# earth-insights/ZoomEarth

Hardware: AMD Instinct MI355X
Metric: questions/sec end-to-end, ZoomEarth-3B on 5000px tiles (higher is better)
Workload: dtype bf16

## Files before the change

### include/zoomearth.h

```cpp
#ifndef ZOOMEARTH_H
#define ZOOMEARTH_H

#include <stddef.h>
#include <stdint.h>

#ifdef __cplusplus
extern "C" {
#endif

typedef struct ze_engine ze_engine;

typedef enum {
    ZE_OK = 0,
    ZE_ERR_INVALID = -1,
    ZE_ERR_HIP = -2,
    ZE_ERR_NOMEM = -3,
    ZE_ERR_NOTFOUND = -4,
    ZE_ERR_MISMATCH = -5
} ze_status;

typedef enum { ZE_F32 = 0, ZE_F16 = 1, ZE_BF16 = 2 } ze_dtype;

#define ZE_MAX_FULLATT 16
#define ZE_MAX_EOS 4
// ... 199 lines not shown
int ze_weight_format(ze_engine* e);

int ze_op_linear(ze_engine* e, const void* a_bf16, const void* w_bf16, const void* bias_bf16, void* c_bf16, int M,
                 int N, int K, int act, void* stream);
int ze_op_gemm(ze_engine* e, int launcher, int epi, const void* a_bf16, int lda, const void* w_bf16, int ldw, const void* bias_bf16,
               const void* r_bf16, int ldr, void* c, int ldc, const int32_t* c_rows, int M, int N, int K, void* stream);
int ze_op_rmsnorm(ze_engine* e, const void* x_bf16, const void* weight_bf16, void* y_bf16, int rows, int cols,
                  float eps, void* stream);
int ze_op_token_logprob(ze_engine* e, const void* logits_bf16, int rows, int vocab, int ld, const int32_t* targets,
                        float* out, void* stream);
int ze_op_score_detail(ze_engine* e, const void* logits_bf16, int rows, int vocab, int ld, const int32_t* targets, int top_n,
                       float* out_logprob, float* out_entropy, int32_t* out_rank, int32_t* out_top_ids, float* out_top_logprobs,
                       void* stream);
int ze_op_attention(ze_engine* e, const void* q, const void* k, const void* v, void* o, int T, int heads,
                    int kv_heads, int D, const int32_t* cu_seqlens, int n_seg, int causal, void* stream);

int ze_op_window_gather(ze_engine* e, const float* pixel_values, const int32_t* grid_thw, int n_images, void* out_bf16, void* stream);
int ze_op_window_scatter(ze_engine* e, const void* x_bf16, int cols, const int32_t* grid_thw, int n_images, void* out_bf16,
                         void* stream);
int ze_op_vision_rope(ze_engine* e, void* qkv_bf16, const int32_t* grid_thw, int n_images, int window_order, void* stream);
int ze_op_embed_scatter(ze_engine* e, const int32_t* input_ids, int len, const void* image_embeds, int n_image_rows, void* out_bf16,
                        void* stream);
int ze_op_mrope_kv(ze_engine* e, int seq, int layer, void* qkv_bf16, int T, const int32_t* position_ids, int past, void* stream);
int ze_op_rope_kv_decode(ze_engine* e, const int32_t* seqs, int n, int layer, void* qkv_bf16, void* stream);
int ze_op_kv_read(ze_engine* e, int seq, int layer, int start, int n, void* out_k, void* out_v, void* stream);

int ze_seq_set_speculation(ze_engine* e, int seq, int k, int min_ngram, int max_ngram, const int32_t* prompt_ids, int n_prompt, void* stream);
int ze_chain_spec_stats(ze_engine* e, int seq, int* steps, int* drafted, int* accepted, void* stream);
int ze_op_spec_draft(ze_engine* e, const int32_t* hist_ids, const int32_t* hist_lens, int rows, int ld, int k, int min_ngram,
                     int max_ngram, int32_t* out_draft, int32_t* out_len, void* stream);
int ze_op_spec_accept(ze_engine* e, const float* logits, int n_chains, int vocab, int ld, int k, const int32_t* draft,
                      const int32_t* draft_len, uint8_t* seen, const float* repetition_penalty, const int32_t* room, int ignore_eos,
                      int32_t* out_tokens, int32_t* out_count, int32_t* out_finished, void* stream);
int ze_op_decode_rows(ze_engine* e, int seq, const int32_t* tokens, int r, float* out_logits, void* stream);
int ze_op_attn_decode(ze_engine* e, const int32_t* seqs, int n, int layer, const void* qkv_bf16, void* out_bf16, void* stream);
int ze_op_attn_decode_single(ze_engine* e, int seq, int layer, const void* qkv_bf16, void* out_bf16, void* stream);
int ze_op_gemv(ze_engine* e, int epi, const void* w_bf16, const void* w8, const void* scale8, const void* x_bf16, const void* norm_w,
               float eps, const void* bias_bf16, int act8, int N, int K, void* out_bf16, float* out_f32, const uint8_t* seen,
               float penalty, int32_t* out_token, int seq, int layer, const void* embed, int token, void* embed_out, void* stream);
int ze_op_logits_rows(ze_engine* e, const void* w_bf16, const void* norm_w, float eps, const void* x_bf16, float* out_f32, int n, int N,
                      int K, void* stream);

int ze_op_numeric_helpers(ze_engine* e, const float* x, const float* y, uint32_t* out, uint32_t* out2, int n, void* stream);

int ze_profile_decode_kernel(ze_engine* e, int which, int iters, float* avg_us, double* bytes_per_launch,
                             void* stream);
int ze_profile_batch_kernel(ze_engine* e, int which, int n, int iters, float* avg_us, double* bytes_per_launch,
                            void* stream);
int ze_profile_prefill_kernel(ze_engine* e, int which, int rows, int iters, float* avg_us, double* flops_per_launch,
                              void* stream);
int ze_profile_prefill_layer(ze_engine* e, int rows, int layers_run, float avg_us[4], double flops[4], void* stream);
int ze_tune(int knob, int value);
int ze_phase_timers(ze_engine* e, int enable, int reset, float out_ms[5]);

#ifdef __cplusplus
}
#endif
#endif
```

### zoomearth_amd/_lib.py

```python
from __future__ import annotations

import ctypes as C
import os
import subprocess

_HERE = os.path.dirname(os.path.abspath(__file__))
LIB_PATH = os.environ.get("ZE_LIB_PATH") or os.path.join(_HERE, "libzoomearth_hip.so")
CSRC = os.path.join(_HERE, "csrc")

ZE_F32, ZE_F16, ZE_BF16 = 0, 1, 2
ZE_MAX_FULLATT, ZE_MAX_EOS = 16, 4


class ZeConfig(C.Structure):
    _fields_ = [
        ("vit_depth", C.c_int32), ("vit_hidden", C.c_int32), ("vit_heads", C.c_int32),
        ("vit_intermediate", C.c_int32), ("vit_out_hidden", C.c_int32),
        ("patch_size", C.c_int32), ("temporal_patch_size", C.c_int32), ("spatial_merge_size", C.c_int32),
        ("window_size", C.c_int32), ("in_channels", C.c_int32),
        ("n_fullatt", C.c_int32), ("fullatt_block_indexes", C.c_int32 * ZE_MAX_FULLATT),
        ("hidden", C.c_int32), ("layers", C.c_int32), ("heads", C.c_int32), ("kv_heads", C.c_int32),
        ("intermediate", C.c_int32), ("vocab", C.c_int32),
        ("rms_eps", C.c_float), ("rope_theta", C.c_float), ("mrope_section", C.c_int32 * 3),
        ("tie_word_embeddings", C.c_int32),
# ... 138 lines not shown
                                          C.POINTER(C.c_float), C.c_int, C.c_int, C.POINTER(C.c_int32), _P]),
    "ze_op_token_logprobs": (C.c_int, [_P, _P, C.c_int, C.c_int, C.c_int, _P, C.c_int, _P, _P, _P, _P]),
    "ze_seq_set_logit_adjust": (C.c_int, [_P, C.c_int, C.c_float, C.c_float, C.c_int, C.POINTER(C.c_int32), C.POINTER(C.c_float),
                                          C.c_int, _P]),
    "ze_op_logit_adjust": (C.c_int, [_P, _P, C.c_int, C.c_int, C.c_int, _P, _P, _P, _P, _P, _P, _P, _P, _P]),
    "ze_seq_set_token_rules": (C.c_int, [_P, C.c_int, C.c_int, C.POINTER(C.c_int32), C.c_int, C.POINTER(C.c_int32), C.c_int,
                                         C.POINTER(C.c_int32), C.c_int, _P]),
    "ze_op_token_rules": (C.c_int, [_P, _P, C.c_int, C.c_int, C.c_int, _P, _P, _P, _P, _P, _P, _P, _P, _P, _P, _P, _P]),
    "ze_grammar_create": (C.c_int, [_P, C.POINTER(C.c_uint16), C.c_int, C.POINTER(C.c_int16), C.c_int, C.POINTER(C.c_uint8),
                                    C.POINTER(C.c_int), _P]),
    "ze_grammar_destroy": (C.c_int, [_P, C.c_int]),
    "ze_seq_set_grammar": (C.c_int, [_P, C.c_int, C.c_int, C.c_int, _P]),
    "ze_chain_grammar_state": (C.c_int, [_P, C.c_int, C.POINTER(C.c_int), C.POINTER(C.c_int), _P]),
    "ze_op_grammar_mask": (C.c_int, [_P, C.c_int, _P, C.c_int, C.c_int, C.c_int, _P, _P, _P]),
    "ze_op_grammar_advance": (C.c_int, [_P, C.c_int, _P, _P, C.c_int, _P, _P]),
    "ze_weights_quantize_fp8": (C.c_int, [_P, _P]),
    "ze_set_fp8_activations": (C.c_int, [_P, C.c_int]),
    "ze_op_quantize_fp8": (C.c_int, [_P, _P, C.c_int, C.c_int, _P, _P, _P]),
    "ze_weights_quantize_mxfp4": (C.c_int, [_P, _P]),
    "ze_op_quantize_mxfp4": (C.c_int, [_P, _P, C.c_int, C.c_int, _P, _P, _P]),
    "ze_op_gemv4": (C.c_int, [_P, C.c_int, _P, _P, _P, _P, C.c_float, _P, C.c_int, C.c_int, _P, _P, _P, C.c_float,
                              C.POINTER(C.c_int32), C.c_int, C.c_int, _P, C.c_int, _P, _P]),
    "ze_weight_format": (C.c_int, [_P]),
    "ze_op_linear_mx": (C.c_int, [_P, _P, _P, _P, _P, _P, _P, C.c_int, C.c_int, C.c_int, C.c_int, _P]),
    "ze_op_linear": (C.c_int, [_P, _P, _P, _P, _P, C.c_int, C.c_int, C.c_int, C.c_int, _P]),
    "ze_op_gemm": (C.c_int, [_P, C.c_int, C.c_int, _P, C.c_int, _P, C.c_int, _P, _P, C.c_int, _P, C.c_int, _P, C.c_int, C.c_int,
                             C.c_int, _P]),
    "ze_op_rmsnorm": (C.c_int, [_P, _P, _P, _P, C.c_int, C.c_int, C.c_float, _P]),
    "ze_op_attention": (C.c_int, [_P, _P, _P, _P, _P, C.c_int, C.c_int, C.c_int, C.c_int, C.POINTER(C.c_int32),
                                  C.c_int, C.c_int, _P]),
    "ze_op_window_gather": (C.c_int, [_P, _P, C.POINTER(C.c_int32), C.c_int, _P, _P]),
    "ze_op_window_scatter": (C.c_int, [_P, _P, C.c_int, C.POINTER(C.c_int32), C.c_int, _P, _P]),
    "ze_op_vision_rope": (C.c_int, [_P, _P, C.POINTER(C.c_int32), C.c_int, C.c_int, _P]),
    "ze_op_embed_scatter": (C.c_int, [_P, C.POINTER(C.c_int32), C.c_int, _P, C.c_int, _P, _P]),
    "ze_op_mrope_kv": (C.c_int, [_P, C.c_int, C.c_int, _P, C.c_int, C.POINTER(C.c_int32), C.c_int, _P]),
    "ze_op_rope_kv_decode": (C.c_int, [_P, C.POINTER(C.c_int32), C.c_int, C.c_int, _P, _P]),
    "ze_op_attn_decode": (C.c_int, [_P, C.POINTER(C.c_int32), C.c_int, C.c_int, _P, _P, _P]),
    "ze_op_attn_decode_single": (C.c_int, [_P, C.c_int, C.c_int, _P, _P, _P]),
    "ze_op_kv_read": (C.c_int, [_P, C.c_int, C.c_int, C.c_int, C.c_int, _P, _P, _P]),
    "ze_seq_set_speculation": (C.c_int, [_P, C.c_int, C.c_int, C.c_int, C.c_int, C.POINTER(C.c_int32), C.c_int, _P]),
    "ze_chain_spec_stats": (C.c_int, [_P, C.c_int, C.POINTER(C.c_int), C.POINTER(C.c_int), C.POINTER(C.c_int), _P]),
    "ze_op_spec_draft": (C.c_int, [_P, _P, _P, C.c_int, C.c_int, C.c_int, C.c_int, C.c_int, _P, _P, _P]),
    "ze_op_spec_accept": (C.c_int, [_P, _P, C.c_int, C.c_int, C.c_int, C.c_int, _P, _P, _P, _P, _P, C.c_int, _P, _P, _P, _P]),
    "ze_op_decode_rows": (C.c_int, [_P, C.c_int, C.POINTER(C.c_int32), C.c_int, _P, _P]),
    "ze_op_gemv": (C.c_int, [_P, C.c_int, _P, _P, _P, _P, _P, C.c_float, _P, C.c_int, C.c_int, C.c_int, _P, _P, _P, C.c_float,
                             C.POINTER(C.c_int32), C.c_int, C.c_int, _P, C.c_int, _P, _P]),
    "ze_op_logits_rows": (C.c_int, [_P, _P, _P, C.c_float, _P, _P, C.c_int, C.c_int, C.c_int, _P]),
    "ze_op_numeric_helpers": (C.c_int, [_P, _P, _P, _P, _P, C.c_int, _P]),
    "ze_profile_decode_kernel": (C.c_int, [_P, C.c_int, C.c_int, C.POINTER(C.c_float), C.POINTER(C.c_double), _P]),
    "ze_profile_batch_kernel": (C.c_int, [_P, C.c_int, C.c_int, C.c_int, C.POINTER(C.c_float), C.POINTER(C.c_double), _P]),
    "ze_profile_prefill_kernel": (C.c_int, [_P, C.c_int, C.c_int, C.c_int, C.POINTER(C.c_float), C.POINTER(C.c_double), _P]),
    "ze_profile_prefill_layer": (C.c_int, [_P, C.c_int, C.c_int, C.POINTER(C.c_float), C.POINTER(C.c_double), _P]),
    "ze_phase_timers": (C.c_int, [_P, C.c_int, C.c_int, C.POINTER(C.c_float)]),
    "ze_tune": (C.c_int, [C.c_int, C.c_int]),
}
EXPORTS = tuple(_SIGS)


def lib():
    global _lib
    if _lib is not None:
        return _lib
    if not os.path.exists(LIB_PATH):
        raise ImportError(
            f"{LIB_PATH} is missing: build it with `python -c 'import __graft_entry__ as g; g.build()'` "
            "(or `make -C zoomearth_amd/csrc`). zoomearth_amd has no CPU fallback.")
    try:
        import torch
    except Exception:
        pass
    handle = C.CDLL(LIB_PATH, mode=C.RTLD_GLOBAL)
    for name, (res, args) in _SIGS.items():
        fn = getattr(handle, name)
        fn.restype = res
        fn.argtypes = args
    _lib = handle
    return _lib


def check(code: int, engine=None):
    if code < 0:
        msg = lib().ze_last_error(engine)
        raise ZoomEarthError(code, msg.decode("utf-8", "replace") if msg else "")
    return code
```

### zoomearth_amd/csrc/ze_engine.h

```cpp
#pragma once
#include <algorithm>
#include <map>
#include <tuple>
#include <set>
#include <string>
#include <vector>

#include "ze_host.h"
#include "ze_kernels.h"

struct ze_linear {
    bf16_t* w = nullptr;
    bf16_t* bias = nullptr;
    int n = 0, k = 0, ld = 0;
    uint8_t* w8 = nullptr;
    float* scale8 = nullptr;
    int ld8 = 0;
    uint8_t* w4 = nullptr;
    uint8_t* scale4 = nullptr;
    bf16_t* wf = nullptr;
    bf16_t* wp = nullptr;
    bf16_t* bias_p = nullptr;
    uint8_t* wf8 = nullptr;
};
// ... 203 lines not shown
    size_t fe_tmp_bytes = 0, fe_img_bytes = 0, fe_coef_ints = 0;
    int* fe_coef_host = nullptr;
    hipEvent_t v_staged = nullptr, t_staged = nullptr;
    hipEvent_t fe_done = nullptr;
    bool fe_in_flight = false;

    bf16_t *vx = nullptr, *vh = nullptr, *vy = nullptr, *vqkv = nullptr, *vo = nullptr, *va = nullptr, *vz = nullptr,
           *vz2 = nullptr;
    float *vcos = nullptr, *vsin = nullptr;
    int *vperm = nullptr, *vinv = nullptr;
    int4* vtiles_win = nullptr;
    int4* vtiles_full = nullptr;
    int* v_host_ints = nullptr;
    float* v_host_f32 = nullptr;
    size_t v_host_ints_cap = 0, v_host_f32_cap = 0;

    bf16_t *th = nullptr, *ty = nullptr, *tqkv = nullptr, *to = nullptr, *ta = nullptr;
    int *tsrc = nullptr, *tpos = nullptr;
    int4* ttiles = nullptr;
    int* ttile_aux = nullptr;
    int* trow_aux = nullptr;
    int* tscore = nullptr;
    int prefill_rows = 0;
    int* t_host_ints = nullptr;
    size_t t_host_ints_cap = 0;
    int *xs_host = nullptr, *xs_dev = nullptr, *xt_host = nullptr, *xt_dev = nullptr;
    size_t xs_cap = 0, xt_cap = 0;
    int *xl_host = nullptr, *xl_dev = nullptr;
    size_t xl_cap = 0;
    hipEvent_t xs_staged = nullptr;

    bf16_t *dh = nullptr, *dq = nullptr, *dattn = nullptr, *dact = nullptr;
    float *dlogits = nullptr, *dpartial = nullptr, *dsample = nullptr;
    int max_splits = 64;
    int* d_host_ints = nullptr;
    unsigned* atickets = nullptr;
    unsigned bgraph_epoch = 0;
    float* gslab = nullptr;
    size_t gslab_floats = 0;
    int gticket_cap = 0;
    ze_gemm_ws gemm_ws() const { return ze_gemm_ws{gslab, gslab_floats, gtickets, gticket_cap}; }
    unsigned* gtickets = nullptr;
    float* pslab = nullptr;
    size_t pslab_floats = 0;
    unsigned* ptickets = nullptr;
    int pticket_cap = 0;
    ze_gemm_ws prefill_ws();
    bf16_t *bh = nullptr, *by = nullptr, *bqkv = nullptr, *bo = nullptr, *ba = nullptr;
    int* bseq = nullptr;
    float *blogits = nullptr, *bpartial = nullptr, *bsample = nullptr;
    ze_seq_dev* bstate_host = nullptr;
    std::map<ze_step_key, hipGraphExec_t> bgraphs;
    int live_parts = 0;

    bool timers_on = false;
    bool counted = false;
    struct ev_pair { int phase; hipEvent_t a, b; };
    std::vector<ev_pair> ev_used;
    std::vector<ev_pair> ev_free;
    float phase_ms[5] = {0, 0, 0, 0, 0};

    bf16_t* kc(int layer, int seq) const {
        return kcache + (((size_t)layer * cfg.max_seqs + seq) * cfg.kv_heads) * (size_t)cfg.max_ctx * head_dim;
    }
    bf16_t* vc(int layer, int seq) const {
        return vcache + (((size_t)layer * cfg.max_seqs + seq) * cfg.kv_heads) * (size_t)cfg.max_ctx * head_dim;
    }
};

#define ZE_TRY(x)               \
    do {                        \
        int _r = (x);           \
        if (_r != 0) return _r; \
    } while (0)
#define ZE_KCHECK() ZE_HIP(hipGetLastError())

extern unsigned ze_tune_epoch;
void ze_weights_changed(ze_engine* e);
int ze_engine_build_layout(ze_engine* e);
int ze_timer_begin(ze_engine* e, int phase, hipStream_t s);
void ze_timer_end(ze_engine* e, int handle, hipStream_t s);

template <typename T>
static int dev_alloc(ze_engine* e, T** p, size_t count, bool zero = true) {
    ZE_HIP(hipMalloc((void**)p, std::max<size_t>(count, 1) * sizeof(T)));
    if (zero) ZE_HIP(hipMemset(*p, 0, std::max<size_t>(count, 1) * sizeof(T)));
    return 0;
}
static inline int check_seq(ze_engine* e, int seq) {
    if (!e) return ze_fail(e, ZE_ERR_INVALID, "null engine");
    if (seq < 0 || seq >= e->cfg.max_seqs) return ze_fail(e, ZE_ERR_NOTFOUND, "sequence id out of range");
    return ZE_OK;
}

#pragma GCC visibility push(hidden)
int ze_requests_create(ze_engine* e);
void ze_requests_free(ze_engine* e);
void ze_requests_clear(ze_engine* e, int seq, hipStream_t s);
const float* ze_requests_rows(ze_engine* e, const float* logits, const int* seq_ids, int slot0, int n, hipStream_t s);
void ze_requests_logprobs(ze_engine* e, const float* logits, const int* seq_ids, int slot0, int n, hipStream_t s);
void ze_requests_after_token(ze_engine* e, const float* logits, const int* seq_ids, int slot0, int n, hipStream_t s);
int ze_check_filter(ze_engine* e, int top_k, float top_p, float min_p);
int ze_check_entropy_filter(ze_engine* e, float typical_p, float epsilon_cutoff, float eta_cutoff);
void ze_attach_filters(ze_engine* e, ze_sample_opts& so, bool batch);
float ze_penalty_of(const ze_engine* e, const ze_gen_params* p, int seq);
ze_sample_opts ze_sample_opts_of(ze_engine* e, const ze_gen_params* p, int slot, bool batch = false);
// ... 55 lines not shown
```

### zoomearth_amd/csrc/ze_forward.hip

```cpp
#include <math.h>
#include <cmath>
#include <string.h>

#include <algorithm>

#include "ze_engine.h"

extern int ze_gemv_knobs[24];

static int frontend_acquire(ze_engine* e) {
    if (e->fe_in_flight) {
        ZE_HIP(hipEventSynchronize(e->fe_done));
        e->fe_in_flight = false;
    }
    return ZE_OK;
}
static int frontend_release(ze_engine* e, hipStream_t s) {
    if (!e->fe_done) ZE_HIP(hipEventCreateWithFlags(&e->fe_done, hipEventDisableTiming));
    ZE_HIP(hipEventRecord(e->fe_done, s));
    e->fe_in_flight = true;
    return ZE_OK;
}
static int stage_acquire(ze_engine* e, hipEvent_t& ev) {
    if (ev) ZE_HIP(hipEventSynchronize(ev));
    return ZE_OK;
}
static int stage_release(ze_engine* e, hipEvent_t& ev, hipStream_t s) {
    if (!ev) ZE_HIP(hipEventCreateWithFlags(&ev, hipEventDisableTiming));
    ZE_HIP(hipEventRecord(ev, s));
    return ZE_OK;
}
static int crop_resize(ze_engine* e, const uint8_t* src, int src_h, int src_w, const int32_t box[4], uint8_t* dst,
                       int dst_h, int dst_w, hipStream_t s) {
    const int bx0 = box[0], by0 = box[1];
    const int bw = box[2] - box[0], bh = box[3] - box[1];
    if (bw <= 0 || bh <= 0 || dst_w <= 0 || dst_h <= 0) return ze_fail(e, ZE_ERR_INVALID, "empty crop box or output");
    const bool need_h = bw != dst_w, need_v = bh != dst_h;
    if (!need_h && !need_v) {
        ze_launch_crop(src, src_h, src_w, bx0, by0, dst, dst_h, dst_w, s);
        ZE_KCHECK();
        return ZE_OK;
    }
    ze_coeffs ch, cv;
    size_t ints = 0;
    if (need_h) {
        ze_bicubic_coeffs(bw, dst_w, &ch);
        ints += 2 * (size_t)dst_w + ch.kk.size();
    }
    if (need_v) {
        ze_bicubic_coeffs(bh, dst_h, &cv);
        ints += 2 * (size_t)dst_h + cv.kk.size();
    }
    if (ints > e->fe_coef_ints) return ze_fail(e, ZE_ERR_NOMEM, "bicubic coefficient table exceeds workspace");
    if (need_h && need_v && (size_t)bh * dst_w * 3 > e->fe_tmp_bytes)
        return ze_fail(e, ZE_ERR_NOMEM, "resize intermediate exceeds workspace (max_tile_side)");
    ZE_TRY(frontend_acquire(e));
    int* hp = e->fe_coef_host;
// ... 1100 lines not shown
static int op_sample(ze_engine* e, int seq, const float* logits, float repetition_penalty, const ze_sample_opts& so,
                     int index, int32_t* out_token, hipStream_t s) {
    ZE_TRY(check_seq(e, seq));
    if (!logits || !out_token) return ze_fail(e, ZE_ERR_INVALID, "null argument");
    if (index < 0 || index >= e->cfg.max_ctx) return ze_fail(e, ZE_ERR_INVALID, "index out of range");
    const ze_config& c = e->cfg;
    hipSetDevice(e->device);
    e->logits_fresh[seq] = 0;
    ZE_TRY(push_state(e, seq, s, 0, 0, 0));
    if (index) ze_launch_set_ints(&(e->st_dev + seq)->n_gen, &index, 1, s);
    ze_launch_sample(logits, c.vocab, e->seen + (size_t)seq * c.vocab, repetition_penalty, e->st_dev + seq, e->eos_dev,
                     c.n_eos, c.pad_token_id, 1, 0, e->out_tokens + (size_t)seq * c.max_ctx, e->dsample, so, s);
    ze_requests_logprobs(e, logits, nullptr, seq, 1, s);
    ZE_KCHECK();
    ZE_HIP(hipMemcpyAsync(out_token, e->out_tokens + (size_t)seq * c.max_ctx + index, sizeof(int), hipMemcpyDeviceToHost, s));
    ZE_HIP(hipStreamSynchronize(s));
    return ZE_OK;
}

extern "C" int ze_op_sample_greedy(ze_engine* e, int seq, const float* logits, float repetition_penalty,
                                   int32_t* out_token, void* stream) {
    return op_sample(e, seq, logits, repetition_penalty, ze_sample_opts{}, 0, out_token, (hipStream_t)stream);
}

extern "C" int ze_op_sample_temperature(ze_engine* e, int seq, const float* logits, float repetition_penalty,
                                        float temperature, uint64_t seed, int index, int32_t* out_token, void* stream) {
    if (!(temperature > 0.f)) return ze_fail(e, ZE_ERR_INVALID, "temperature must be positive");
    ze_sample_opts so;
    so.temperature = temperature;
    so.seed = seed;
    so.slot = seq;
    if (check_seq(e, seq) == 0) ze_attach_filters(e, so, false);
    return op_sample(e, seq, logits, repetition_penalty, so, index, out_token, (hipStream_t)stream);
}

template <typename F>
static int capture_step(ze_engine* e, F enqueue, hipGraphExec_t* exec) {
    hipStream_t cs;
    ZE_HIP(hipStreamCreateWithFlags(&cs, hipStreamNonBlocking));
    hipGraph_t graph = nullptr;
    int r = ZE_OK;
    if (hipStreamBeginCapture(cs, hipStreamCaptureModeThreadLocal) != hipSuccess)
        r = ze_fail(e, ZE_ERR_HIP, "hipStreamBeginCapture failed");
    if (r == ZE_OK) r = enqueue(cs);
    if (hipStreamEndCapture(cs, &graph) != hipSuccess && r == ZE_OK)
        r = ze_fail(e, ZE_ERR_HIP, "hipStreamEndCapture failed");
    if (r == ZE_OK && hipGraphInstantiate(exec, graph, nullptr, nullptr, 0) != hipSuccess)
        r = ze_fail(e, ZE_ERR_HIP, "hipGraphInstantiate failed");
    if (graph) hipGraphDestroy(graph);
    hipStreamDestroy(cs);
    return r;
}

static int first_token(ze_engine* e, int q, float pen, int ign, const ze_sample_opts& so, hipStream_t s) {
    const ze_config& c = e->cfg;
    const float* row = e->dlogits + (size_t)q * c.vocab;
    e->logits_fresh[q] = 0;
    ze_launch_sample(ze_requests_rows(e, row, nullptr, q, 1, s), c.vocab, e->seen + (size_t)q * c.vocab, pen, e->st_dev + q, e->eos_dev,
                     c.n_eos, c.pad_token_id, ign, 0, e->out_tokens + (size_t)q * c.max_ctx, e->dsample, so, s);
    ze_requests_after_token(e, row, nullptr, q, 1, s);
    ZE_KCHECK();
    return ZE_OK;
}

static int trim_at_eos(const ze_config& c, const int32_t* tokens, int n) {
    for (int i = 0; i < n; ++i)
        for (int k = 0; k < c.n_eos; ++k)
            if (tokens[i] == c.eos_token_ids[k]) return i + 1;
    return n;
}

extern "C" int ze_generate(ze_engine* e, int seq, const ze_gen_params* p, int32_t* out_tokens, int* n_out,
                           void* stream) {
    ZE_TRY(check_seq(e, seq));
    if (!p || !out_tokens || !n_out) return ze_fail(e, ZE_ERR_INVALID, "null argument");
    const ze_config& c = e->cfg;
    hipStream_t s = (hipStream_t)stream;
    hipSetDevice(e->device);
    int max_new = p->max_new_tokens;
    if (max_new <= 0) {
        *n_out = 0;
        return ZE_OK;
    }
    if (e->ctx_host[seq] + max_new - 1 > c.max_ctx) max_new = c.max_ctx - e->ctx_host[seq] + 1;
    if (max_new <= 0) return ze_fail(e, ZE_ERR_NOMEM, "sequence exceeds max_ctx");
    const float pen = ze_penalty_of(e, p, seq);
    const int ign = p->ignore_eos ? 1 : 0;
    const ze_sample_opts so = ze_sample_opts_of(e, p, seq);
    int32_t* dev_out = e->out_tokens + (size_t)seq * c.max_ctx;
    ze_seq_dev* st = e->st_dev + seq;

    const int t_s = ze_timer_begin(e, 4, s);
    const int r0 = first_token(e, seq, pen, ign, so, s);
    ze_timer_end(e, t_s, s);
    ZE_TRY(r0);

    hipGraphExec_t gexec = nullptr;
    if (p->use_graph && max_new > 1) {
        const ze_step_key key = ze_step_key_of(e, 0, seq, pen, ign, so);
        if (!e->graphs[seq] || !(e->graph_key[seq] == key)) {
            if (e->graphs[seq]) {
                hipGraphExecDestroy(e->graphs[seq]);
                e->graphs[seq] = nullptr;
            }
            ZE_TRY(capture_step(e, [&](hipStream_t cs) { return ze_enqueue_decode_step(e, seq, pen, ign, true, so, cs); }, &e->graphs[seq]));
            e->graph_key[seq] = key;
// ... 80 lines not shown
            q.kv_heads = c.kv_heads;
        }
        ZE_HIP(hipMemcpyAsync(e->qkv_epi_dev, host.data(), sizeof(ze_qkv_epi) * c.layers, hipMemcpyHostToDevice, s));
        ZE_HIP(hipStreamSynchronize(s));
        ZE_KCHECK();
    }
    if (ok && !wide) {
        const size_t per_layer = (size_t)(nqkv + 2 * ip) * H + (size_t)H * nq;
        const size_t total = per_layer * c.layers + (size_t)c.vocab * H;
        if (!e->arena_f) ZE_HIP(hipMalloc((void**)&e->arena_f, total * sizeof(bf16_t)));
        bf16_t* cur = e->arena_f;
        auto pack = [&](ze_linear& l, int rows, int cols, int rope_dim) {
            ze_launch_pack_fragments(l.w, l.ld, rows, cols, cur, s, rope_dim);
            l.wf = cur;
            cur += (size_t)rows * cols;
        };
        for (int li = 0; li < c.layers; ++li) {
            ze_text_layer& L = e->tl[li];
            pack(L.qkv, nqkv, H, hd);
            pack(L.o, H, nq, 0);
            pack(L.gate_up, 2 * ip, H, 0);
        }
        ze_launch_pack_fragments(e->lm_head, H, c.vocab, H, cur, s);
        e->lm_head_f = cur;
        for (int li = 0; li < c.layers; ++li) {
            ze_text_layer& L = e->tl[li];
            L.qkv.wf8 = L.o.wf8 = L.gate_up.wf8 = nullptr;
        }
        e->lm_head8.wf8 = nullptr;
        if (e->fp8_ready) {
            const bool head8 = e->lm_head8.w8 != nullptr;
            const size_t bytes = ((size_t)(nqkv + 2 * ip) * H + (size_t)H * nq) * c.layers + (head8 ? (size_t)c.vocab * H : 0);
            if (!e->arena_f8) ZE_HIP(hipMalloc((void**)&e->arena_f8, bytes));
            uint8_t* c8 = e->arena_f8;
            auto pack8 = [&](ze_linear& l, int rows, int cols, int rope_dim) {
                ze_launch_pack_fragments8(l.w8, l.ld8, rows, cols, c8, s, rope_dim);
                l.wf8 = c8;
                c8 += (size_t)rows * cols;
            };
            for (int li = 0; li < c.layers; ++li) {
                ze_text_layer& L = e->tl[li];
                pack8(L.qkv, nqkv, H, hd);
                pack8(L.o, H, nq, 0);
                pack8(L.gate_up, 2 * ip, H, 0);
            }
            if (head8) pack8(e->lm_head8, c.vocab, H, 0);
        }
        ZE_KCHECK();
    }
    e->frag_ready = true;
    return ZE_OK;
}

void set_live_parts(ze_engine* e, const int32_t* seqs, int n, int steps) {
    int mx = 0, ml = 0;
    for (int i = 0; i < n; ++i) {
        const int c = e->ctx_host[seqs[i]] + std::max(1, steps) + 1, sp = e->split_host[seqs[i]];
        mx = std::max(mx, e->ctx_host[seqs[i]]);
        ml = std::max(ml, (sp + 383) / 384 + (c - sp + 383) / 384);
    }
    e->live_parts = (mx + std::max(1, steps) + 1 + 191) / 192;
    e->live_parts_long = ml;
}

void upload_mates(ze_engine* e, const int32_t* seqs, int n, hipStream_t s) {
    std::vector<int> mate(n, -1);
    if (e->prefix_hints && ze_gemv_knobs[17] != 1) {
        std::map<long long, int> open;
        for (int i = 0; i < n; ++i) {
            const int q = seqs[i], sp = e->split_host[q];
            if (sp <= 0) continue;
            const int h = e->pfx_pushed[q];
            const int holder = (h != 0 && (h & 0xffff) >= sp) ? (h >> 16) : q;
            const long long key = ((long long)holder << 20) | (long long)sp;
            auto it = open.find(key);
            if (it == open.end()) open[key] = i;
            else {
                mate[i] = it->second;
                mate[it->second] = i;
                open.erase(it);
            }
        }
    }
    ze_launch_set_ints(e->bmate, mate.data(), n, s);
}

static int upload_batch(ze_engine* e, const int32_t* seqs, int n, hipStream_t s) {
    if (n <= 0 || n > e->cfg.max_seqs) return ze_fail(e, ZE_ERR_INVALID, "batch size out of range");
    if (n > 64 && !e->wide_regime())
        return ze_fail(e, ZE_ERR_INVALID, "more than 64 chains in a step of an engine pinned to the fragment kernels (ze_set_decode_regime)");
    for (int i = 0; i < n; ++i) {
        if (seqs[i] < 0 || seqs[i] >= e->cfg.max_seqs) return ze_fail(e, ZE_ERR_NOTFOUND, "sequence id out of range");
        for (int j = 0; j < i; ++j)
            if (seqs[j] == seqs[i]) return ze_fail(e, ZE_ERR_INVALID, "duplicate sequence id in a batch");
        if (e->ctx_host[seqs[i]] + 1 > e->cfg.max_ctx) return ze_fail(e, ZE_ERR_NOMEM, "sequence exceeds max_ctx");
    }
    ze_launch_set_ints(e->bseq, seqs, n, s);
    sync_prefix(e, seqs, n, s);
    upload_mates(e, seqs, n, s);
    return ZE_OK;
}

static bool attn_per_wave(const ze_engine* e) {
    const ze_config& c = e->cfg;
    const int wparts = (c.max_ctx + 191) / 192;
    return ze_gemv_knobs[8] != 2 && ze_gemv_knobs[11] == 0 && wparts <= std::max(e->max_splits, 8) && wparts <= 64 && e->head_dim == 128 &&
           c.heads / c.kv_heads <= 16;
}

static void launch_batch_attention(ze_engine* e, int li, int n, bool frag_out, hipStream_t s, const bf16_t* q_rows = nullptr,
                                   bf16_t* out_rows = nullptr) {
    const ze_config& c = e->cfg;
    const int hd = e->head_dim, nq = c.heads * hd, nqkv = nq + 2 * c.kv_heads * hd;
    const size_t seq_stride = (size_t)c.kv_heads * c.max_ctx * hd;
    const float scale = 1.0f / sqrtf((float)hd);
    const bf16_t* qb = q_rows ? q_rows : e->bqkv;
    bf16_t* ob = out_rows ? out_rows : e->bo;
    if (e->brow_off && !q_rows) {
// ... 128 lines not shown
    return false;
}

static int enqueue_decode_batch(ze_engine* e, int n, float penalty, int ignore_eos, int sample, const ze_sample_opts& so,
                                hipStream_t s) {
    const ze_config& c = e->cfg;
    ze_launch_embed_tokens_batch(e->st_dev, e->bseq, n, e->embed, e->bh, c.hidden, s);
    for (int li = 0; li < c.layers; ++li) {
        batch_norm(e, li, n, ZE_NORM_IN, s);
        batch_qkv(e, li, n, s);
        batch_attention(e, li, n, s);
        batch_o(e, li, n, s);
        batch_norm(e, li, n, ZE_NORM_POST, s);
        batch_gate_up(e, li, n, s);
        batch_down(e, li, n, s);
    }
    batch_norm(e, 0, n, ZE_NORM_FINAL, s);
    batch_lm_head(e, 0, n, s);
    ze_launch_sample_batch(sample ? ze_requests_rows(e, e->blogits, e->bseq, 0, n, s) : e->blogits, c.vocab, e->seen, penalty, e->st_dev,
                           e->bseq, n, e->eos_dev, c.n_eos, c.pad_token_id, ignore_eos, 1, sample, e->out_tokens, c.max_ctx, e->bsample,
                           e->bsample + (size_t)c.max_seqs * 2 * 128, so, s);
    if (sample) ze_requests_after_token(e, e->blogits, e->bseq, 0, n, s);
    ZE_KCHECK();
    return ZE_OK;
}

extern "C" int ze_decode_batch(ze_engine* e, const int32_t* seqs, int n, const int32_t* tokens, float* out_logits,
                               void* stream) {
    if (!e || !seqs) return ze_fail(e, ZE_ERR_INVALID, "null argument");
    const ze_config& c = e->cfg;
    hipStream_t s = (hipStream_t)stream;
    hipSetDevice(e->device);
    ZE_TRY(ensure_fragments(e, s));
    ZE_TRY(upload_batch(e, seqs, n, s));
    set_live_parts(e, seqs, n, 1);
    for (int i = 0; i < n; ++i) e->logits_fresh[seqs[i]] = 0;
    if (tokens) {
        for (int i = 0; i < n; ++i) {
            if (tokens[i] >= c.vocab) return ze_fail(e, ZE_ERR_INVALID, "token id out of range");
            if (tokens[i] >= 0) ze_launch_set_ints(&(e->st_dev + seqs[i])->token, &tokens[i], 1, s);
        }
    }
    const int th = ze_timer_begin(e, 3, s);
    ZE_TRY(enqueue_decode_batch(e, n, 1.0f, 1, 0, ze_sample_opts{}, s));
    ze_timer_end(e, th, s);
    for (int i = 0; i < n; ++i) e->ctx_host[seqs[i]] += 1;
    if (out_logits)
        ZE_HIP(hipMemcpyAsync(out_logits, e->blogits, (size_t)n * c.vocab * sizeof(float), hipMemcpyDeviceToDevice, s));
    return ZE_OK;
}

static int batch_step_graph(ze_engine* e, int na, float pen, int ign, const ze_sample_opts& bso, hipGraphExec_t* out) {
    const ze_step_key key = ze_step_key_of(e, na, 0, pen, ign, bso);
    if (e->bgraph_epoch != ze_tune_epoch) {
        for (auto& kv : e->bgraphs) hipGraphExecDestroy(kv.second);
        e->bgraphs.clear();
        e->bgraph_epoch = ze_tune_epoch;
    }
    auto it = e->bgraphs.find(key);
    if (it == e->bgraphs.end()) {
        hipGraphExec_t ex = nullptr;
        ZE_TRY(capture_step(e, [&](hipStream_t cs) { return enqueue_decode_batch(e, na, pen, ign, 1, bso, cs); }, &ex));
        it = e->bgraphs.emplace(key, ex).first;
    }
    *out = it->second;
    return ZE_OK;
}

static int run_burst(ze_engine* e, const std::vector<int>& active, int steps, const ze_gen_params* p, float pen, int ign,
                     const ze_sample_opts& bso, hipStream_t s) {
    const int na = (int)active.size();
    ZE_TRY(upload_batch(e, active.data(), na, s));
    set_live_parts(e, active.data(), na, steps);
    hipGraphExec_t gx = nullptr;
    if (p->use_graph) ZE_TRY(batch_step_graph(e, na, pen, ign, bso, &gx));
    for (int i = 0; i < steps; ++i) {
        if (gx)
            ZE_HIP(hipGraphLaunch(gx, s));
        else
            ZE_TRY(enqueue_decode_batch(e, na, pen, ign, 1, bso, s));
    }
    for (int q : active) e->ctx_host[q] += steps, e->logits_fresh[q] = 0;
    return ZE_OK;
}

struct spec_layout {
    int rows = 0, n_plain = 0, n_chains = 0;
};

static bool spec_step_ok(const ze_engine* e) {
    const batch_regime r = regime_of(e, 0);
    const int k8 = ze_gemv_knobs[8], k23 = ze_gemv_knobs[23];
    return r.fr && r.fl && attn_per_wave(e) && k8 != 1 && k8 != 4 && k23 != 2 && k23 != 3;
}

static void enqueue_rows_forward(ze_engine* e, int n, hipStream_t s) {
    const ze_config& c = e->cfg;
    ze_spec& q = e->spec;
    struct rows_buffers {
        ze_engine* e;
        int* bseq;
        float *blogits, *bpartial;
        unsigned* atickets;
        explicit rows_buffers(ze_engine* e_) : e(e_), bseq(e_->bseq), blogits(e_->blogits), bpartial(e_->bpartial), atickets(e_->atickets) {
            const ze_spec& q = e->spec;
            e->bseq = q.row_seq, e->blogits = q.logits, e->bpartial = q.partial, e->atickets = q.tickets, e->brow_off = q.row_off;
        }
        ~rows_buffers() { e->bseq = bseq, e->blogits = blogits, e->bpartial = bpartial, e->atickets = atickets, e->brow_off = nullptr; }
        rows_buffers(const rows_buffers&) = delete;
        rows_buffers& operator=(const rows_buffers&) = delete;
    } guard(e);
    ze_launch_spec_embed(q.row_tok, n, e->embed, e->bh, c.hidden, s);
    for (int li = 0; li < c.layers; ++li) {
        batch_norm(e, li, n, ZE_NORM_IN, s);
        batch_qkv(e, li, n, s);
        batch_attention(e, li, n, s);
        batch_o(e, li, n, s);
        batch_norm(e, li, n, ZE_NORM_POST, s);
        batch_gate_up(e, li, n, s);
// ... 14 lines not shown
    enqueue_rows_forward(e, L.rows, s);
    if (L.n_plain > 0) {
        ze_launch_sample_batch(ze_requests_rows(e, q.logits, q.row_seq, 0, L.n_plain, s), c.vocab, e->seen, penalty, e->st_dev, q.row_seq,
                               L.n_plain, e->eos_dev, c.n_eos, c.pad_token_id, ign, 1, 1, e->out_tokens, c.max_ctx, e->bsample,
                               e->bsample + (size_t)c.max_seqs * 2 * 128, so, s);
        ze_requests_after_token(e, q.logits, q.row_seq, 0, L.n_plain, s);
    }
    ze_launch_spec_accept(a, L.n_plain, s);
    ZE_KCHECK();
    return ZE_OK;
}

static int spec_burst(ze_engine* e, const std::vector<int>& chains, int steps, const ze_gen_params* p, float pen, int ign, hipStream_t s) {
    const ze_config& c = e->cfg;
    ze_spec& q = e->spec;
    if (e->wide_regime() || !spec_step_ok(e))
        return ze_fail(e, ZE_ERR_INVALID, "a speculative burst needs the fragment kernels and the pipelined decode attention (family 0, default ze_tune knobs)");
    for (size_t i = 0; i < chains.size(); ++i) {
        for (size_t j = 0; j < i; ++j)
            if (chains[i] == chains[j]) return ze_fail(e, ZE_ERR_INVALID, "duplicate sequence id in a batch");
        if (q.on(chains[i]) && q.pending[chains[i]])
            return ze_fail(e, ZE_ERR_INVALID, "a speculating chain of this burst has a burst in flight: ze_decode_burst_end first");
        if (!q.on(chains[i]) && e->ctx_host[chains[i]] > c.max_ctx) return ze_fail(e, ZE_ERR_NOMEM, "sequence exceeds max_ctx");
    }
    const bool call_draws = p->do_sample && p->temperature > 0.f;
    std::vector<int> order;
    for (int pass = 0; pass < 2; ++pass)
        for (int ch : chains)
            if ((int)q.on(ch) == pass) order.push_back(ch);
    spec_layout L;
    std::vector<int> row_seq, tab;
    int mx = 0;
    for (int ch : order) {
        const int k = q.on(ch) ? q.host[ch].k : 0;
        const ze_chain_sampling& own = e->req.samp_host[ch];
        if (k > 0 && (own.penalty > 0.f ? own.temperature > 0.f : call_draws))
            return ze_fail(e, ZE_ERR_INVALID, "speculation is greedy only: the burst samples a speculating chain");
        if (k == 0) steps = std::min(steps, c.max_ctx - e->ctx_host[ch]);
        const float cp = own.penalty > 0.f ? own.penalty : pen;
        int bits;
        memcpy(&bits, &cp, sizeof(bits));
        tab.insert(tab.end(), {ch, L.rows, k + 1, bits});
        for (int j = 0; j <= k; ++j) row_seq.push_back(ch);
        L.rows += k + 1;
        L.n_chains += 1;
        if (k == 0) L.n_plain += 1;
    }
    if (L.rows > ZE_SP_MAX_ROWS) return ze_fail(e, ZE_ERR_INVALID, "more than 64 rows in a speculative step (one per plain chain, k + 1 per speculating chain)");
    if (steps <= 0) return 0;
    for (int ch : chains) mx = std::max(mx, std::min(c.max_ctx, e->ctx_host[ch] + steps * ((q.on(ch) ? q.host[ch].k : 0) + 1) + 1));
    ze_launch_set_ints(q.row_seq, row_seq.data(), L.rows, s);
    ze_launch_set_ints(q.chains, tab.data(), (int)tab.size(), s);
    sync_prefix(e, chains.data(), (int)chains.size(), s);
    e->live_parts = (mx + 191) / 192;
    e->live_parts_long = (mx + 383) / 384;
    const ze_sample_opts bso = ze_sample_opts_of(e, p, 0, true);
    hipGraphExec_t gx = nullptr;
    if (p->use_graph) {
        ze_step_key key = ze_step_key_of(e, L.rows, 0, pen, ign, bso);
        key.n = L.rows | L.n_plain << 8 | L.n_chains << 16 | 1 << 30;
        if (e->bgraph_epoch != ze_tune_epoch) {
            for (auto& kv : e->bgraphs) hipGraphExecDestroy(kv.second);
            e->bgraphs.clear();
            e->bgraph_epoch = ze_tune_epoch;
        }
        auto it = e->bgraphs.find(key);
        if (it == e->bgraphs.end()) {
            hipGraphExec_t ex = nullptr;
            ZE_TRY(capture_step(e, [&](hipStream_t cs) { return enqueue_spec_step(e, L, pen, ign, bso, cs); }, &ex));
            it = e->bgraphs.emplace(key, ex).first;
        }
        gx = it->second;
    }
    for (int i = 0; i < steps; ++i) {
        if (gx)
            ZE_HIP(hipGraphLaunch(gx, s));
        else
            ZE_TRY(enqueue_spec_step(e, L, pen, ign, bso, s));
    }
    for (int ch : chains) {
        if (!q.on(ch)) e->ctx_host[ch] += steps;
        else q.pending[ch] = 1;
        e->logits_fresh[ch] = 0;
    }
    return steps;
}

extern "C" int ze_op_decode_rows(ze_engine* e, int seq, const int32_t* tokens, int r, float* out_logits, void* stream) {
    ZE_TRY(check_seq(e, seq));
    const ze_config& c = e->cfg;
    if (!tokens || r < 1) return ze_fail(e, ZE_ERR_INVALID, "null tokens or r < 1");
    if (r > ZE_SP_MAX_ROWS) return ze_fail(e, ZE_ERR_INVALID, "more than 64 rows in a step");
    for (int j = 0; j < r; ++j)
        if (tokens[j] < 0 || tokens[j] >= c.vocab) return ze_fail(e, ZE_ERR_INVALID, "token id out of range");
    if (e->ctx_host[seq] + r > c.max_ctx) return ze_fail(e, ZE_ERR_NOMEM, "sequence exceeds max_ctx");
    hipSetDevice(e->device);
    hipStream_t s = (hipStream_t)stream;
    ZE_TRY(ensure_fragments(e, s));
    if (e->wide_regime() || !spec_step_ok(e))
        return ze_fail(e, ZE_ERR_INVALID, "rows of one chain need the fragment kernels and the pipelined decode attention (family 0, default ze_tune knobs)");
    ZE_TRY(ze_spec_alloc(e));
    ze_spec& q = e->spec;
    std::vector<int> row_seq(r, seq), row_off(r);
    for (int j = 0; j < r; ++j) row_off[j] = j;
    ze_launch_set_ints(q.row_seq, row_seq.data(), r, s);
    ze_launch_set_ints(q.row_off, row_off.data(), r, s);
    ze_launch_set_ints(q.row_tok, tokens, r, s);
    sync_prefix(e, &seq, 1, s);
    e->live_parts = (e->ctx_host[seq] + r + 191) / 192;
    e->live_parts_long = (e->ctx_host[seq] + r + 383) / 384;
    enqueue_rows_forward(e, r, s);
    e->ctx_host[seq] += r;
    e->logits_fresh[seq] = 0;
    e->tok_host[seq] = tokens[r - 1];
    ze_launch_set_ints(&(e->st_dev + seq)->ctx, &e->ctx_host[seq], 1, s);
    ze_launch_set_ints(&(e->st_dev + seq)->token, &tokens[r - 1], 1, s);
    ZE_KCHECK();
    if (out_logits) ZE_HIP(hipMemcpyAsync(out_logits, q.logits, (size_t)r * c.vocab * sizeof(float), hipMemcpyDeviceToDevice, s));
    return ZE_OK;
}

static int begin_chain(ze_engine* e, int q, const ze_gen_params* p, int ign, int sample_stream, hipStream_t s) {
    const ze_sample_opts so = ze_sample_opts_of(e, p, q);
    if (so.temperature > 0.f) ze_launch_set_ints(&(e->st_dev + q)->stream, &sample_stream, 1, s);
    return first_token(e, q, ze_penalty_of(e, p, q), ign, so, s);
}

extern "C" int ze_generate_batch(ze_engine* e, const int32_t* seqs, int n, const ze_gen_params* p, int32_t* out_tokens,
                                 int32_t* n_out, void* stream) {
    if (!e || !seqs || !p || !out_tokens || !n_out) return ze_fail(e, ZE_ERR_INVALID, "null argument");
    const ze_config& c = e->cfg;
    hipStream_t s = (hipStream_t)stream;
    hipSetDevice(e->device);
    const int max_new = p->max_new_tokens;
    if (max_new <= 0 || n <= 0) return ze_fail(e, ZE_ERR_INVALID, "max_new_tokens and n must be positive");
    ZE_TRY(ensure_fragments(e, s));
    std::vector<int> limit(c.max_seqs, 0);
    for (int i = 0; i < n; ++i) {
        if (seqs[i] < 0 || seqs[i] >= c.max_seqs) return ze_fail(e, ZE_ERR_NOTFOUND, "sequence id out of range");
        for (int j = 0; j < i; ++j)
            if (seqs[j] == seqs[i]) return ze_fail(e, ZE_ERR_INVALID, "duplicate sequence id in a batch");
        if (e->ctx_host[seqs[i]] > c.max_ctx) return ze_fail(e, ZE_ERR_NOMEM, "sequence exceeds max_ctx");
        limit[seqs[i]] = std::min(max_new, c.max_ctx - e->ctx_host[seqs[i]] + 1);
    }
    const float pen = p->repetition_penalty > 0.f ? p->repetition_penalty : 1.0f;
    const int ign = p->ignore_eos ? 1 : 0;
    const ze_sample_opts bso = ze_sample_opts_of(e, p, 0, true);
    for (int i = 0; i < n; ++i) ZE_TRY(begin_chain(e, seqs[i], p, ign, i, s));
    std::vector<int> active;
    std::vector<int> produced(c.max_seqs, 0);
    for (int i = 0; i < n; ++i) {
        produced[seqs[i]] = 1;
        if (limit[seqs[i]] > 1) active.push_back(seqs[i]);
    }
    const int sync_every = std::max(1, p->sync_every);
    const int td = ze_timer_begin(e, 3, s);
    int steps = 1;
    while (steps < max_new && !active.empty()) {
        int burst = std::min(sync_every, max_new - steps);
        for (int q : active) burst = std::min(burst, limit[q] - produced[q]);
        ZE_TRY(run_burst(e, active, burst, p, pen, ign, bso, s));
        steps += burst;
        for (int q : active) produced[q] += burst;
// ... 887 lines not shown
```

Measured before the change: 71.08.

## Centralize batch graph caching and set only the attention extent each kernel uses

Moves the two duplicated graph-cache lookups into one helper that also counts captures and replays and the time spent capturing, exposed through a new stats entry point. Replaces the direct live_parts/live_parts_long assignments with a function that sets only the extent the selected attention kernel variant reads and zeroes the other. Split-prefix mate uploads and split-part accounting are skipped unless the split knob is on. The live-part values likely feed graph keys or kernel grid sizes, so this can reduce graph recaptures and per-step host work, but it risks wrong extents if a kernel still reads the zeroed field.

```diff
diff --git a/include/zoomearth.h b/include/zoomearth.h
--- a/include/zoomearth.h
+++ b/include/zoomearth.h
@@ -275,6 +275,7 @@
 int ze_profile_prefill_layer(ze_engine* e, int rows, int layers_run, float avg_us[4], double flops[4], void* stream);
 int ze_tune(int knob, int value);
 int ze_phase_timers(ze_engine* e, int enable, int reset, float out_ms[5]);
+int ze_decode_graph_stats(ze_engine* e, int64_t* captured, int64_t* replayed, double* capture_ms);
 
 #ifdef __cplusplus
 }
diff --git a/zoomearth_amd/_lib.py b/zoomearth_amd/_lib.py
--- a/zoomearth_amd/_lib.py
+++ b/zoomearth_amd/_lib.py
@@ -214,6 +214,7 @@
     "ze_profile_prefill_kernel": (C.c_int, [_P, C.c_int, C.c_int, C.c_int, C.POINTER(C.c_float), C.POINTER(C.c_double), _P]),
     "ze_profile_prefill_layer": (C.c_int, [_P, C.c_int, C.c_int, C.POINTER(C.c_float), C.POINTER(C.c_double), _P]),
     "ze_phase_timers": (C.c_int, [_P, C.c_int, C.c_int, C.POINTER(C.c_float)]),
+    "ze_decode_graph_stats": (C.c_int, [_P, C.POINTER(C.c_int64), C.POINTER(C.c_int64), C.POINTER(C.c_double)]),
     "ze_tune": (C.c_int, [C.c_int, C.c_int]),
 }
 EXPORTS = tuple(_SIGS)
diff --git a/zoomearth_amd/csrc/ze_engine.h b/zoomearth_amd/csrc/ze_engine.h
--- a/zoomearth_amd/csrc/ze_engine.h
+++ b/zoomearth_amd/csrc/ze_engine.h
@@ -279,6 +279,8 @@
     ze_seq_dev* bstate_host = nullptr;
     std::map<ze_step_key, hipGraphExec_t> bgraphs;
     int live_parts = 0;
+    int64_t graphs_captured = 0, graphs_replayed = 0;
+    double graph_capture_ms = 0;
 
     bool timers_on = false;
     bool counted = false;
diff --git a/zoomearth_amd/csrc/ze_forward.hip b/zoomearth_amd/csrc/ze_forward.hip
--- a/zoomearth_amd/csrc/ze_forward.hip
+++ b/zoomearth_amd/csrc/ze_forward.hip
@@ -3,6 +3,7 @@
 #include <string.h>
 
 #include <algorithm>
+#include <chrono>
 
 #include "ze_engine.h"
 
@@ -1209,6 +1210,35 @@
     return r;
 }
 
+template <typename F>
+static int batch_graph_of(ze_engine* e, const ze_step_key& key, F enqueue, hipGraphExec_t* out) {
+    if (e->bgraph_epoch != ze_tune_epoch) {
+        for (auto& kv : e->bgraphs) hipGraphExecDestroy(kv.second);
+        e->bgraphs.clear();
+        e->bgraph_epoch = ze_tune_epoch;
+    }
+    auto it = e->bgraphs.find(key);
+    if (it == e->bgraphs.end()) {
+        const auto t0 = std::chrono::steady_clock::now();
+        hipGraphExec_t ex = nullptr;
+        ZE_TRY(capture_step(e, enqueue, &ex));
+        it = e->bgraphs.emplace(key, ex).first;
+        e->graphs_captured += 1;
+        e->graph_capture_ms += std::chrono::duration<double, std::milli>(std::chrono::steady_clock::now() - t0).count();
+    } else
+        e->graphs_replayed += 1;
+    *out = it->second;
+    return ZE_OK;
+}
+
+extern "C" int ze_decode_graph_stats(ze_engine* e, int64_t* captured, int64_t* replayed, double* capture_ms) {
+    if (!e) return ze_fail(e, ZE_ERR_INVALID, "null argument");
+    if (captured) *captured = e->graphs_captured;
+    if (replayed) *replayed = e->graphs_replayed;
+    if (capture_ms) *capture_ms = e->graph_capture_ms;
+    return ZE_OK;
+}
+
 static int first_token(ze_engine* e, int q, float pen, int ign, const ze_sample_opts& so, hipStream_t s) {
     const ze_config& c = e->cfg;
     const float* row = e->dlogits + (size_t)q * c.vocab;
@@ -1395,18 +1425,40 @@
     return ZE_OK;
 }
 
+static bool attn_per_wave(const ze_engine* e);
+static bool split_knob() { return ze_gemv_knobs[23] == 2 || ze_gemv_knobs[23] == 3; }
+
+static void set_attn_extents(ze_engine* e, int parts192, int parts384, bool rows) {
+    const int max_ctx = e->cfg.max_ctx, k8 = ze_gemv_knobs[8];
+    const int wparts = (max_ctx + 191) / 192, lparts = (max_ctx + 383) / 384;
+    e->live_parts = e->live_parts_long = 0;
+    if (rows)
+        e->live_parts_long = std::min(lparts, std::max(1, parts384));
+    else if (k8 == 1 || k8 == 3 || !attn_per_wave(e))
+        ;
+    else if (k8 == 4)
+        e->live_parts = std::min(wparts, std::max(1, parts192));
+    else if (split_knob() && lparts + 1 <= wparts)
+        e->live_parts_long = std::min(lparts + 1, std::max(1, parts384));
+    else
+        e->live_parts = 2 * std::min(lparts, std::max(1, (parts192 + 1) / 2));
+}
+
 void set_live_parts(ze_engine* e, const int32_t* seqs, int n, int steps) {
+    const bool split = split_knob();
     int mx = 0, ml = 0;
     for (int i = 0; i < n; ++i) {
-        const int c = e->ctx_host[seqs[i]] + std::max(1, steps) + 1, sp = e->split_host[seqs[i]];
+        const int c = e->ctx_host[seqs[i]] + std::max(1, steps) + 1;
         mx = std::max(mx, e->ctx_host[seqs[i]]);
+        if (!split) continue;
+        const int sp0 = e->split_host[seqs[i]], sp = (sp0 > 0 && sp0 < c) ? sp0 : 0;
         ml = std::max(ml, (sp + 383) / 384 + (c - sp + 383) / 384);
     }
-    e->live_parts = (mx + std::max(1, steps) + 1 + 191) / 192;
-    e->live_parts_long = ml;
+    set_attn_extents(e, (mx + std::max(1, steps) + 1 + 191) / 192, ml, false);
 }
 
 void upload_mates(ze_engine* e, const int32_t* seqs, int n, hipStream_t s) {
+    if (!split_knob()) return;
     std::vector<int> mate(n, -1);
     if (e->prefix_hints && ze_gemv_knobs[17] != 1) {
         std::map<long long, int> open;
@@ -1641,19 +1693,7 @@
 
 static int batch_step_graph(ze_engine* e, int na, float pen, int ign, const ze_sample_opts& bso, hipGraphExec_t* out) {
     const ze_step_key key = ze_step_key_of(e, na, 0, pen, ign, bso);
-    if (e->bgraph_epoch != ze_tune_epoch) {
-        for (auto& kv : e->bgraphs) hipGraphExecDestroy(kv.second);
-        e->bgraphs.clear();
-        e->bgraph_epoch = ze_tune_epoch;
-    }
-    auto it = e->bgraphs.find(key);
-    if (it == e->bgraphs.end()) {
-        hipGraphExec_t ex = nullptr;
-        ZE_TRY(capture_step(e, [&](hipStream_t cs) { return enqueue_decode_batch(e, na, pen, ign, 1, bso, cs); }, &ex));
-        it = e->bgraphs.emplace(key, ex).first;
-    }
-    *out = it->second;
-    return ZE_OK;
+    return batch_graph_of(e, key, [&](hipStream_t cs) { return enqueue_decode_batch(e, na, pen, ign, 1, bso, cs); }, out);
 }
 
 static int run_burst(ze_engine* e, const std::vector<int>& active, int steps, const ze_gen_params* p, float pen, int ign,
@@ -1774,25 +1814,13 @@
     ze_launch_set_ints(q.row_seq, row_seq.data(), L.rows, s);
     ze_launch_set_ints(q.chains, tab.data(), (int)tab.size(), s);
     sync_prefix(e, chains.data(), (int)chains.size(), s);
-    e->live_parts = (mx + 191) / 192;
-    e->live_parts_long = (mx + 383) / 384;
+    set_attn_extents(e, 0, (mx + 383) / 384, true);
     const ze_sample_opts bso = ze_sample_opts_of(e, p, 0, true);
     hipGraphExec_t gx = nullptr;
     if (p->use_graph) {
         ze_step_key key = ze_step_key_of(e, L.rows, 0, pen, ign, bso);
         key.n = L.rows | L.n_plain << 8 | L.n_chains << 16 | 1 << 30;
-        if (e->bgraph_epoch != ze_tune_epoch) {
-            for (auto& kv : e->bgraphs) hipGraphExecDestroy(kv.second);
-            e->bgraphs.clear();
-            e->bgraph_epoch = ze_tune_epoch;
-        }
-        auto it = e->bgraphs.find(key);
-        if (it == e->bgraphs.end()) {
-            hipGraphExec_t ex = nullptr;
-            ZE_TRY(capture_step(e, [&](hipStream_t cs) { return enqueue_spec_step(e, L, pen, ign, bso, cs); }, &ex));
-            it = e->bgraphs.emplace(key, ex).first;
-        }
-        gx = it->second;
+        ZE_TRY(batch_graph_of(e, key, [&](hipStream_t cs) { return enqueue_spec_step(e, L, pen, ign, bso, cs); }, &gx));
     }
     for (int i = 0; i < steps; ++i) {
         if (gx)
@@ -1829,8 +1857,7 @@
     ze_launch_set_ints(q.row_off, row_off.data(), r, s);
     ze_launch_set_ints(q.row_tok, tokens, r, s);
     sync_prefix(e, &seq, 1, s);
-    e->live_parts = (e->ctx_host[seq] + r + 191) / 192;
-    e->live_parts_long = (e->ctx_host[seq] + r + 383) / 384;
+    set_attn_extents(e, 0, (e->ctx_host[seq] + r + 383) / 384, true);
     enqueue_rows_forward(e, r, s);
     e->ctx_host[seq] += r;
     e->logits_fresh[seq] = 0;
```

Result: slower. 69.13 (-2.8%).
